# HengyiWang/MorpheuS

Hardware: AMD Instinct MI355X
Metric: rays/sec (fwd+bwd, 128 samples/ray) (higher is better)
Workload: dtype f32 (exact 3 x bf16 operand split on the bf16 MFMA pipe, fp32 accumulate)

## Files before the change

include/morpheus_hip.h:

```cpp
#ifndef MORPHEUS_HIP_H
#define MORPHEUS_HIP_H

#include <stdint.h>

#ifdef __cplusplus
extern "C" {
#endif

#define MH_OK 0
#define MH_ERR_ARG 1
#define MH_ERR_LAUNCH 2
#define MH_ERR_OVERFLOW 3

#define MH_ABI_VERSION 9
#define MH_MAX_LEVELS 32
#define MH_TILE 32

int mh_abi_version(void);
const char *mh_status_string(int status);

int mh_grid_encode_fwd(const float *x, const float *emb, const int32_t *offsets_host,
                       const int32_t *res_host, float *out, int64_t M, int32_t L, int32_t n_levels,
                       float bound, int32_t group, void *stream);
int mh_grid_encode_bwd(const float *grad, const float *x, const float *emb,
// ... 102 lines not shown
int64_t mh_field_wpack_floats(void);
int64_t mh_field_wpackT_floats(void);
int mh_field_fwd(const float *xc, const float *feat_s, const float *feat_c, const float *topo,
                 const float *wpack, const float *bias, const float *beta, int32_t n_bands, int32_t with_color,
                 float *sdf, float *sigma, float *albedo, float *acts, int64_t M, void *stream);
int64_t mh_mlp_wgrad_workspace_floats(int32_t n_layers, const int32_t *in_feats_host,
                                      const int32_t *out_feats_host, int64_t n_tiles);
int mh_mlp_wgrad(const float *acts, const float *dpre, int64_t acts_tile_floats, int64_t dpre_tile_floats,
                 int32_t n_layers, const int32_t *act_off_host, const int32_t *dpre_off_host,
                 const int32_t *in_feats_host, const int32_t *out_feats_host, const int32_t *in_live_host,
                 const int32_t *out_live_host, float *workspace, float *dw_raw, float *db_raw, int64_t n_tiles, void *stream);
int mh_mlp_wgrad_b3(const float *acts, const float *dpre, int64_t acts_tile_floats, int64_t dpre_tile_floats,
                    int32_t n_layers, const int32_t *act_off_host, const int32_t *dpre_off_host,
                    const int32_t *in_feats_host, const int32_t *out_feats_host, const int32_t *in_live_host,
                    const int32_t *out_live_host, float *workspace, float *dw_raw, float *db_raw, int64_t n_tiles, void *stream);

int mh_weight_norm_fwd(int32_t n_layers, const float *const *v_host, const float *const *g_host, float *const *w_host,
                       const int32_t *rows_host, const int32_t *cols_host, void *stream);
int mh_weight_norm_bwd(int32_t n_layers, const float *const *v_host, const float *const *g_host,
                       const float *const *dw_host, float *const *dv_host, float *const *dg_host,
                       const int32_t *rows_host, const int32_t *cols_host, void *stream);

int64_t mh_field_bwd_fused_workspace_floats(int64_t M);
int64_t mh_field_dgeo_floats(int64_t M);
int mh_field_bwd_fused(const float *xc, const float *sdf, const float *albedo, const float *g_sdf, const float *g_sigma,
                       const float *g_albedo, const float *wpackT, const float *beta, int32_t n_bands, int32_t with_color,
                       const float *acts, float *dgeo_scratch, float *workspace, float *raw, int32_t accumulate, float *g_xc,
                       float *g_feat_s, float *g_feat_c, float *g_topo, uint32_t *gmax_bits, int64_t M, void *stream);
int64_t mh_field_w3T_bytes(void);
int mh_field_bwd_fused_b3(const float *xc, const float *sdf, const float *albedo, const float *g_sdf, const float *g_sigma,
                          const float *g_albedo, const void *w3T, const float *beta, int32_t n_bands, int32_t with_color,
                          const float *acts, float *dgeo_scratch, float *workspace, float *raw, int32_t accumulate, float *g_xc,
                          float *g_feat_s, float *g_feat_c, float *g_topo, uint32_t *gmax_bits, int64_t M, void *stream);
int mh_adam_step(float *params, const float *grads, float *exp_avg, float *exp_avg_sq, int64_t n, int32_t n_segs,
                 const int64_t *seg_end_host, const float *seg_lr_host, const int64_t *seg_step_host, float beta1,
                 float beta2, float eps, void *stream);
int mh_adam_step_dev(float *params, const float *grads, float *exp_avg, float *exp_avg_sq, int64_t n, int32_t n_segs,
                     const int64_t *seg_end_host, const float *seg_lr_host, const float *seg_flag_dev, int64_t *seg_step_dev,
                     float *seg_scratch_dev, float beta1, float beta2, float eps, void *stream);

int64_t mh_masked_mean_workspace_floats(void);
int mh_masked_mean_fwd(int32_t kind, const float *a, const float *b, const float *w_row, int64_t M, int32_t C,
                       const int32_t *n_valid, float *ws, float *out, void *stream);
int mh_masked_mean_bwd(int32_t kind, const float *a, const float *b, const float *w_row, int64_t M, int32_t C,
                       const int32_t *n_valid, const float *out, const float *g, float *g_a, float *g_b, void *stream);
int mh_ortho_perturb_fwd(const float *x, const float *n, const float *phi, float scale, int64_t M, float *out, void *stream);
int mh_ortho_perturb_bwd(const float *n, const float *phi, const float *g_out, float scale, int64_t M, float *g_n, void *stream);
int mh_smooth_points_fwd(const float *depth, const float *off, const float *rays_o, const float *rays_d, int64_t N, int32_t K,
                         float *pts, float *keep, void *stream);
int mh_smooth_points_bwd(const float *g_pts, const float *depth, const float *off, const float *rays_d, int64_t N, int32_t K,
                         float *g_depth, float *g_o, float *g_d, void *stream);
int mh_bg_blend_fwd(const float *color, const float *opacity, const float *bg, int64_t N, float *image, void *stream);
int mh_bg_blend_bwd(const float *g_image, const float *opacity, const float *bg, int64_t N, float *g_opacity, float *g_bg, void *stream);

int64_t mh_pose_bwd_workspace_floats(int64_t B, int64_t n_per_row);
int mh_pose_apply_fwd(const float *rays_o, const float *rays_d, const float *pose, const int64_t *frame_of_row, int64_t B,
                      int64_t n_per_row, float *o_out, float *d_out, void *stream);
int mh_pose_apply_bwd(const float *rays_d, const float *pose, const int64_t *frame_of_row, int64_t B, int64_t n_per_row,
                      int64_t n_frames, const float *g_o, const float *g_d, float *ws, float *g_pose, void *stream);

int mh_render_loss_fwd(const float *pred_rgb, const float *pred_depth, const float *opacity, const float *image,
                       const float *depth, const float *mask, const float *bg, const float *rays_o, const float *rays_d,
                       int64_t N, float w_rgb, float w_mask, float w_depth, float *gt_rgb, float *valid, float *out, void *stream);
int mh_render_loss_bwd(const float *pred_rgb, const float *pred_depth, const float *opacity, const float *gt_rgb,
                       const float *depth, const float *mask, const float *valid, int64_t N, float w_rgb, float w_mask,
                       float w_depth, const float *g, float *g_rgb, float *g_depth, float *g_opacity, void *stream);
// ... 98 lines not shown
```

morpheus_amd/csrc/mlp.hip:

```cpp
#include "mlp_dev.h"
#include <stdlib.h>


__shared__ f32x4 lds_w[4096];

template <int N_F4>
__device__ __forceinline__ void stage_weights(const float *__restrict__ g) {
    static_assert(N_F4 % 256 == 0, "whole rounds of the 256-thread block");
    __syncthreads();
    const f32x4 *src = reinterpret_cast<const f32x4 *>(g);
    const int wave = threadIdx.x >> 6;
#pragma unroll
    for (int k = 0; k < N_F4 / 256; k++)
        __builtin_amdgcn_global_load_lds((const __attribute__((address_space(1))) void *)(src + k * 256 + threadIdx.x),
                                         (__attribute__((address_space(3))) void *)(lds_w + k * 256 + wave * 64), 16, 0, 0);
    asm volatile("s_waitcnt vmcnt(0)" ::: "memory");
    __syncthreads();
}

template <int N_F4>
__device__ __forceinline__ void stage_issue(const float *__restrict__ g) {
    static_assert(N_F4 % 256 == 0, "whole rounds of the 256-thread block");
    const f32x4 *src = reinterpret_cast<const f32x4 *>(g);
    const int wave = threadIdx.x >> 6;
#pragma unroll
    for (int k = 0; k < N_F4 / 256; k++)
        __builtin_amdgcn_global_load_lds((const __attribute__((address_space(1))) void *)(src + k * 256 + threadIdx.x),
                                         (__attribute__((address_space(3))) void *)(lds_w + k * 256 + wave * 64), 16, 0, 0);
}
__device__ __forceinline__ void stage_wait() {
    asm volatile("s_waitcnt vmcnt(0)" ::: "memory");
    __syncthreads();
}

// ... 1043 lines not shown
                wsdf[mt] += q[(7 + mt) * 64 + lane];
            }
            gb_acc += q[6 * 64 + lane];
        }
    }
    if (wave != 0) return;
#pragma unroll
    for (int o = 32; o > 0; o >>= 1) gb_acc += __shfl_xor(gb_acc, o);
    if (lane == 0) ws[part.gb + blockIdx.x] = gb_acc;
    const int64_t pchunk = blockIdx.x;
#pragma unroll
    for (int mt = 0; mt < 2; mt++) {
        dw_store<3>(ws + part.dw[0] + pchunk * 64 * 96, w0[mt], mt, 96, i, h);
        dw_store<2>(ws + part.dw[1] + pchunk * 64 * 64, w1[mt], mt, 64, i, h);
    }
    {
        f32x16 z[2];
        acc_zero<2>(z);
        if (!WITH_COLOR) dw_store<2>(ws + part.dw[2] + pchunk * 64 * 64, z, 0, 64, i, h);
        if (h == 0) {
            z[0][0] = wsdf[0];
            z[1][0] = wsdf[1];
        }
        dw_store<2>(ws + part.dw[2] + pchunk * 64 * 64, z, 1, 64, i, h);
    }
    if (h == 0) {
        if (!WITH_COLOR) ws[part.db[2] + pchunk * 64 + i] = 0.f;
        ws[part.db[2] + pchunk * 64 + 32 + i] = i == 0 ? bsdf : 0.f;
#pragma unroll
        for (int mt = 0; mt < 2; mt++) {
            ws[part.db[1] + pchunk * 64 + 32 * mt + i] = b1[mt];
            ws[part.db[0] + pchunk * 64 + 32 * mt + i] = b0[mt];
        }
    }
}

template <int IT>
struct WgFrag {
    f32x4 a[4];
    f32x4 b[IT][4];
};

__device__ __forceinline__ int wg_row(int row, int live) { return row < live ? row : live - 1; }

template <int IT>
__device__ __forceinline__ void wg_load(WgFrag<IT> &f, const float *__restrict__ acts, const float *__restrict__ dpre,
                                        int64_t t, int64_t acts_tile_floats, int64_t dpre_tile_floats, int act_off,
                                        int dpre_off, int mt, int i, int h, int in_live, int out_live) {
    const f32x4 *a = reinterpret_cast<const f32x4 *>(dpre + t * dpre_tile_floats + dpre_off + (int64_t)wg_row(32 * mt + i, out_live) * TILE + 16 * h);
#pragma unroll
    for (int j = 0; j < 4; j++) f.a[j] = a[j];
#pragma unroll
    for (int n = 0; n < IT; n++) {
        const f32x4 *b = reinterpret_cast<const f32x4 *>(acts + t * acts_tile_floats + act_off + (int64_t)wg_row(32 * n + i, in_live) * TILE + 16 * h);
#pragma unroll
        for (int j = 0; j < 4; j++) f.b[n][j] = b[j];
    }
}

template <int IT>
__device__ __forceinline__ void wg_load_async(WgFrag<IT> &f, const float *__restrict__ acts, const float *__restrict__ dpre,
                                              int64_t t, int64_t acts_tile_floats, int64_t dpre_tile_floats, int act_off,
                                              int dpre_off, int mt, int i, int h, int in_live, int out_live) {
    const float *a = dpre + t * dpre_tile_floats + dpre_off + (int64_t)wg_row(32 * mt + i, out_live) * TILE + 16 * h;
    asm volatile("global_load_dwordx4 %0, %1, off" : "=v"(f.a[0]) : "v"(a) : "memory");
    asm volatile("global_load_dwordx4 %0, %1, off offset:16" : "=v"(f.a[1]) : "v"(a) : "memory");
// ... 888 lines not shown
    const WarpWg w = warp_wg_geometry();
    WgRegenHost rg;
    for (int k = 0; k < WG_MAX_LAYERS; k++) rg.on[k] = false;
    rg.M = M;
    for (int net = 0; net < 2; net++) {
        const int k = net * 6 + 4;
        rg.on[k] = regen_dpre4 != 0;
        rg.g5[k] = net ? g_topo : g_deform;
        rg.nout[k] = net ? 2 : 3;
        rg.w3T[k] = reinterpret_cast<const f32x4 *>(net ? w3T_t : w3T_d);
        rg.mask_off[k] = WARP_HID_ROWS * TILE + (net * 5 + 4) * 64 * 2;
    }
    return wgrad_impl(acts, dpre, (int64_t)WARP_ACT_ROWS * TILE, (int64_t)WARP_DPRE_ROWS * TILE, 12, w.act_off, w.dpre_off, w.in, w.out,
                      w.in_live, w.out_live, workspace, dw_raw, db_raw, n_tiles_for(M), stream, true, regen_dpre4 ? &rg : nullptr);
}

static const int FUSED_IN[6] = {96, 64, 64, 64, 64, 64};
static const int FUSED_OUT[6] = {64, 64, 64, 64, 64, 32};

static inline int fused_blocks(int64_t n_tiles) {
    const int64_t need = (n_tiles + FUSED_THREADS / 64 - 1) / (FUSED_THREADS / 64);
    const int64_t cus = mh_cu_count();
    return (int)(need < cus ? need : cus);
}

extern "C" int64_t mh_field_bwd_fused_workspace_floats(int64_t M) {
    const int64_t chunks = (int64_t)fused_blocks(n_tiles_for(M));
    int64_t per = 0;
    for (int l = 0; l < 6; l++) per += (int64_t)FUSED_IN[l] * FUSED_OUT[l] + FUSED_OUT[l];
    return chunks * (per + 1);
}
extern "C" int64_t mh_field_dgeo_floats(int64_t M) { return n_tiles_for(M) * 64 * 16; }

static int field_bwd_fused_impl(const float *xc, const float *sdf, const float *albedo, const float *g_sdf,
                                const float *g_sigma, const float *g_albedo, const float *wpackT, const float *beta,
                                int32_t n_bands, int32_t with_color, const float *acts, float *dgeo_scratch,
                                float *workspace, float *raw, int32_t accumulate, float *g_xc, float *g_feat_s, float *g_feat_c,
                                float *g_topo, uint32_t *gmax_bits, int64_t M, void *stream, bool b3) {
    if (M == 0) return MH_OK;
    if (M < 0 || !xc || !sdf || !wpackT || !acts || !workspace || !raw || n_bands < 0 || n_bands > 6 || !beta) return MH_ERR_ARG;
    if (with_color && (!albedo || !dgeo_scratch)) return MH_ERR_ARG;
    static MhOncePerDevice opted;
    const size_t lds_c = (size_t)(FUSED_TC2(b3) + FUSED_TC1(b3) + FUSED_TC0(b3)) * 16 + (size_t)(4 * SCR_FLOATS) * sizeof(float);
    const size_t lds_s = (size_t)(FUSED_TS2(b3) + FUSED_TS1(b3) + FUSED_TS0(b3)) * 16 + (size_t)(4 * SCR_FLOATS) * sizeof(float);
    const int dev = mh_device();
    if (opted.need(dev)) {
        const int big_c = (int)((size_t)(FUSED_TC2(1) + FUSED_TC1(1) + FUSED_TC0(1)) * 16 + (size_t)(4 * SCR_FLOATS) * sizeof(float));
        const int big_s = (int)((size_t)(FUSED_TS2(1) + FUSED_TS1(1) + FUSED_TS0(1)) * 16 + (size_t)(4 * SCR_FLOATS) * sizeof(float));
        if (hipFuncSetAttribute((const void *)field_fused_color_kernel<false>, hipFuncAttributeMaxDynamicSharedMemorySize, big_c) != hipSuccess ||
            hipFuncSetAttribute((const void *)field_fused_color_kernel<true>, hipFuncAttributeMaxDynamicSharedMemorySize, big_c) != hipSuccess ||
            hipFuncSetAttribute((const void *)field_fused_sdf_kernel<true, false>, hipFuncAttributeMaxDynamicSharedMemorySize, big_s) != hipSuccess ||
            hipFuncSetAttribute((const void *)field_fused_sdf_kernel<false, false>, hipFuncAttributeMaxDynamicSharedMemorySize, big_s) != hipSuccess ||
            hipFuncSetAttribute((const void *)field_fused_sdf_kernel<true, true>, hipFuncAttributeMaxDynamicSharedMemorySize, big_s) != hipSuccess ||
            hipFuncSetAttribute((const void *)field_fused_sdf_kernel<false, true>, hipFuncAttributeMaxDynamicSharedMemorySize, big_s) != hipSuccess)
            return MH_ERR_LAUNCH;
        opted.mark(dev);
    }
    const int64_t n_tiles = n_tiles_for(M);
    const int blocks = fused_blocks(n_tiles);
    const int64_t chunks = blocks;
    int64_t dw_off[6], db_off[6], off = 0, dw_total = 0, db_total = 0;
    for (int l = 0; l < 6; l++) {
        dw_off[l] = off;
        off += chunks * FUSED_IN[l] * FUSED_OUT[l];
        dw_total += (int64_t)FUSED_IN[l] * FUSED_OUT[l];
    }
    for (int l = 0; l < 6; l++) {
        db_off[l] = off;
        off += chunks * FUSED_OUT[l];
        db_total += FUSED_OUT[l];
    }
    FusedPart pc, ps;
    for (int k = 0; k < 3; k++) {
        ps.dw[k] = dw_off[k];
        ps.db[k] = db_off[k];
        pc.dw[k] = dw_off[3 + k];
        pc.db[k] = db_off[3 + k];
    }
    ps.gb = off;
    pc.gb = off;
    ps.dw_s2 = pc.dw_s2 = dw_off[2];
    ps.db_s2 = pc.db_s2 = db_off[2];
    hipStream_t st = mh_stream(stream);
#define FUSED_LAUNCH_COLOR(B3_)                                                                                             \
    hipLaunchKernelGGL(field_fused_color_kernel<B3_>, dim3((unsigned)blocks), dim3(FUSED_THREADS), lds_c, st, albedo, g_albedo, wpackT, \
                       acts, dgeo_scratch, g_feat_c, workspace, pc, gmax_bits, M, n_tiles)
#define FUSED_LAUNCH_SDF(WC, B3_, DGEO)                                                                                      \
    hipLaunchKernelGGL((field_fused_sdf_kernel<WC, B3_>), dim3((unsigned)blocks), dim3(FUSED_THREADS), lds_s, st, xc, sdf, g_sdf, \
                       g_sigma, wpackT, beta, (int)n_bands, acts, (const float *)(DGEO), g_xc, g_feat_s, g_topo,             \
                       workspace, ps, gmax_bits, M, n_tiles)
    if (with_color) {
        if (b3) FUSED_LAUNCH_COLOR(true); else FUSED_LAUNCH_COLOR(false);
        MH_CHECK_LAUNCH();
        if (b3) FUSED_LAUNCH_SDF(true, true, dgeo_scratch); else FUSED_LAUNCH_SDF(true, false, dgeo_scratch);
    } else {
        if (b3) FUSED_LAUNCH_SDF(false, true, nullptr); else FUSED_LAUNCH_SDF(false, false, nullptr);
    }
#undef FUSED_LAUNCH_COLOR
#undef FUSED_LAUNCH_SDF
    MH_CHECK_LAUNCH();
    const int n_l = with_color ? 6 : 3;
    WgReduce rd;
    rd.n = 13;
    rd.accumulate = accumulate ? 1 : 0;
    int64_t dw_out = 0, db_out = 0;
    rd.first[0] = 0;
    for (int l = 0; l < 6; l++) {
        const int32_t ch = l < n_l ? (int32_t)chunks : 0;
        rd.chunks[l] = ch;
        rd.len[l] = FUSED_IN[l] * FUSED_OUT[l];
        rd.part_off[l] = dw_off[l];
        rd.out_off[l] = dw_out;
        rd.chunks[6 + l] = ch;
        rd.len[6 + l] = FUSED_OUT[l];
        rd.part_off[6 + l] = db_off[l];
        rd.out_off[6 + l] = dw_total + db_out;
        dw_out += (int64_t)FUSED_IN[l] * FUSED_OUT[l];
        db_out += FUSED_OUT[l];
    }
    rd.chunks[12] = (int32_t)chunks;
    rd.len[12] = 1;
    rd.part_off[12] = ps.gb;
    rd.out_off[12] = dw_total + db_total;
    for (int sgm = 0; sgm < rd.n; sgm++) rd.first[sgm + 1] = rd.first[sgm] + rd.len[sgm];
// ... 39 lines not shown
```

morpheus_amd/ops.py:

```python
from __future__ import annotations

import ctypes
import math
import os
from typing import Optional, Sequence

import numpy as np
import torch

from . import _lib
from ._lib import check, launch, ptr, require_gpu, stream
from .packing import field_joint_packer, field_packer, warp_joint_packer, warp_packer



class KernelTimer:

    def __init__(self):
        self.enabled = False
        self.records = {}
        self._pool, self._used = [], 0

    def reset(self, enabled: bool):
        self.enabled, self.records, self._used = enabled, {}, 0
# ... 847 lines not shown
    for net in range(2):
        for l in range(6):
            act_off.append(0 if l == 0 else (64 + net * 640 + (l - 1) * 128) * 32)
            dpre_off.append((net * 672 + l * 128) * 32)
            in_pad.append(64 if l == 0 else 128)
            out_pad.append(32 if l == 5 else 128)
            in_live.append(40 if l == 0 else 128)
            out_live.append((3, 2)[net] if l == 5 else 128)
    return act_off, dpre_off, in_pad, out_pad, in_live, out_live


_WARP_WG = _warp_wg_geometry()

def warp_mlp(x, slot, bias0_d, bias0_t, n_bands, opnd: MLPOperands, slots_are_identity: bool = False):
    return _WarpMLP.apply(x, slot, bias0_d, bias0_t, opnd.token, n_bands, opnd, slots_are_identity)


def _field_fwd(lib, xc, fs, fc, tp, beta_c, n_bands, with_color, opnd, need_grad):
    w, b = opnd.w[0], opnd.b[0]
    M, dev = xc.shape[0], xc.device
    acts = _scratch(lib.mh_field_acts_floats(M), dev) if need_grad else None
    sdf, sigma = torch.empty(M, device=dev), torch.empty(M, device=dev)
    albedo = torch.empty(M, 3, device=dev) if with_color else None
    if opnd.w3 is not None:
        _timed("mh_field_fwd_b3", ptr(xc), ptr(fs), ptr(fc), ptr(tp), ptr(opnd.w3[0]), ptr(b), ptr(beta_c), n_bands,
               int(bool(with_color)), ptr(sdf), ptr(sigma), ptr(albedo), ptr(acts), M, key="mh_field_fwd")
    else:
        _timed("mh_field_fwd", ptr(xc), ptr(fs), ptr(fc), ptr(tp), ptr(w), ptr(b), ptr(beta_c), n_bands, int(bool(with_color)),
               ptr(sdf), ptr(sigma), ptr(albedo), ptr(acts), M)
    return sdf, sigma, albedo, acts


FIELD_BWD = os.environ.get("MORPHEUS_FIELD_BWD", "b3")
if FIELD_BWD not in ("b3", "sdf", "f32"):
    raise ValueError(f"MORPHEUS_FIELD_BWD={FIELD_BWD!r}: expected 'b3', 'sdf' or 'f32'")


def _field_wT(opnd, with_color: bool):
    sliced = FIELD_BWD == "b3" or (FIELD_BWD == "sdf" and not with_color)
    if sliced and opnd.mode == "b3" and opnd.wT3 is not None:
        return opnd.wT3[0], True
    return opnd.wT[0], False


def _field_bwd(lib, xc, wT, beta_c, acts, sdf, albedo, g_sdf, g_sigma, g_albedo, n_bands, with_color, has_topo, has_fc,
               need_dx, jp, raw_into=None, gmax=None, b3=False):
    M, dev = xc.shape[0], xc.device
    if not with_color:
        g_albedo = None
    g_xc = torch.empty(M, 3, device=dev) if need_dx else None
    g_fs = _scratch(M * 32, dev).view(M, 32)
    g_fc = _scratch(M * 32, dev).view(M, 32) if (with_color and has_fc) else None
    g_tp = torch.empty(M, 2, device=dev) if has_topo else None
    if gmax is None:
        gmax = torch.zeros(2, dtype=torch.int32, device=dev)
    dgeo = _scratch(lib.mh_field_dgeo_floats(M), dev) if with_color else None
    ws = torch.empty(lib.mh_field_bwd_fused_workspace_floats(M), device=dev)
    raw = None
    if raw_into is None:
        raw = torch.empty(jp.raw_len + 1, device=dev) if M > 0 else torch.zeros(jp.raw_len + 1, device=dev)
    c = lambda t: None if t is None else t.contiguous()
    _timed("mh_field_bwd_fused_b3" if b3 else "mh_field_bwd_fused", ptr(xc), ptr(sdf), ptr(albedo if with_color else None), ptr(c(g_sdf)),
           ptr(c(g_sigma)), ptr(c(g_albedo)), ptr(wT), ptr(beta_c), n_bands, int(with_color), ptr(acts), ptr(dgeo), ptr(ws),
           ptr(raw) if raw_into is None else ctypes.c_void_p(raw_into), int(raw_into is not None), ptr(g_xc), ptr(g_fs), ptr(g_fc),
           ptr(g_tp), ptr(gmax), M, key="mh_field_bwd_fused")
    return g_xc, g_fs, g_fc, g_tp, raw, gmax


class _FieldMLP(torch.autograd.Function):

    @staticmethod
    def forward(ctx, xc, feat_s, feat_c, topo, beta, token, n_bands, with_color, opnd):
        ctx.set_materialize_grads(False)
        require_gpu(xc, feat_s, feat_c, topo, beta)
        lib = _lib.load()
        xc = xc.detach().contiguous().float()
        fs = feat_s.detach().contiguous()
        fc = None if feat_c is None else feat_c.detach().contiguous()
        tp = None if topo is None else topo.detach().contiguous()
        beta_c = beta.detach().reshape(1).contiguous().float()
        sdf, sigma, albedo, acts = _field_fwd(lib, xc, fs, fc, tp, beta_c, n_bands, with_color, opnd, any(ctx.needs_input_grad))
        wT_sel, ctx.bwd_b3 = _field_wT(opnd, bool(with_color))
        ctx.save_for_backward(xc, wT_sel, beta_c, acts, sdf, albedo)
        ctx.cfg = (n_bands, bool(with_color), topo is not None, feat_c is not None)
        ctx.jp = opnd.jp
        if albedo is None:
            albedo = torch.empty(0, device=xc.device)
            ctx.mark_non_differentiable(albedo)
        return sdf, sigma, albedo

    @staticmethod
    def backward(ctx, g_sdf, g_sigma, g_albedo):
        lib = _lib.load()
        xc, wT, beta_c, acts, sdf, albedo = ctx.saved_tensors
# ... 388 lines not shown
```

Baseline: 1.062 million.

## Add paired-wave 512-thread field backward kernels splitting output tiles across waves

New measurement: 1.085 million (median of 6 runs). +2.1%, better.

```diff
diff --git a/include/morpheus_hip.h b/include/morpheus_hip.h
--- a/include/morpheus_hip.h
+++ b/include/morpheus_hip.h
@@ -158,6 +158,7 @@
                           const float *g_albedo, const void *w3T, const float *beta, int32_t n_bands, int32_t with_color,
                           const float *acts, float *dgeo_scratch, float *workspace, float *raw, int32_t accumulate, float *g_xc,
                           float *g_feat_s, float *g_feat_c, float *g_topo, uint32_t *gmax_bits, int64_t M, void *stream);
+int64_t mh_field_bwd_pair_min_points(int64_t set);
 int mh_adam_step(float *params, const float *grads, float *exp_avg, float *exp_avg_sq, int64_t n, int32_t n_segs,
                  const int64_t *seg_end_host, const float *seg_lr_host, const int64_t *seg_step_host, float beta1,
                  float beta2, float eps, void *stream);
diff --git a/morpheus_amd/csrc/mlp.hip b/morpheus_amd/csrc/mlp.hip
--- a/morpheus_amd/csrc/mlp.hip
+++ b/morpheus_amd/csrc/mlp.hip
@@ -1,5 +1,6 @@
 #include "mlp_dev.h"
 #include <stdlib.h>
+#include <atomic>
 
 
 __shared__ f32x4 lds_w[4096];
@@ -1109,6 +1110,606 @@
             ws[part.db[1] + pchunk * 64 + 32 * mt + i] = b1[mt];
             ws[part.db[0] + pchunk * 64 + 32 * mt + i] = b0[mt];
         }
+    }
+}
+
+#define PAIR_THREADS 512
+#define PAIR_RED_FLOATS (6 * 1024 + 8 * 64)
+
+#define PAIR_LANE_ANEW                                            \
+    int lane_anew = threadIdx.x & 63;                             \
+    asm volatile("" : "+v"(lane_anew));                           \
+    const int lane = lane_anew, pt = lane & 31, h = lane >> 5, i = lane & 31
+
+struct PairWalk {
+    int64_t chunk, n_chunks, trips;
+};
+__device__ __forceinline__ PairWalk pair_walk(int pair, int64_t n_tiles) {
+    PairWalk w;
+    w.n_chunks = 4 * (int64_t)gridDim.x;
+    const int64_t first = 4 * (int64_t)blockIdx.x;
+    w.chunk = first + pair;
+    w.trips = first < n_tiles ? (n_tiles - first + w.n_chunks - 1) / w.n_chunks : 0;
+    return w;
+}
+
+template <int N_F4>
+__device__ __forceinline__ void stage_pair(const float *__restrict__ g) {
+    const f32x4 *src = reinterpret_cast<const f32x4 *>(g);
+    for (int i = threadIdx.x; i < N_F4; i += PAIR_THREADS) lds_fused[i] = src[i];
+}
+
+__device__ __forceinline__ void scr_put_tile(float *__restrict__ scr, const float (&v)[16], int t, int pt, int h) {
+#pragma unroll
+    for (int r = 0; r < 16; r++) scr[(32 * t + acc_row(r, h)) * SCR_STRIDE + pt] = v[r];
+}
+
+template <int KS, int MT, int NT, int S_RUN = KS / 8>
+__device__ __forceinline__ void mfma_tiles_z_b3(const f32x4 *__restrict__ w, int t0, const float (&bin)[KS], f32x16 (&acc)[NT], int lane) {
+    static_assert(KS % 8 == 0 && S_RUN >= 1 && S_RUN <= KS / 8 && NT <= MT, "k16 steps");
+    constexpr int S = KS / 8, PL = MT * S * 64;
+    const f32x16 zero = {0.f, 0.f, 0.f, 0.f, 0.f, 0.f, 0.f, 0.f, 0.f, 0.f, 0.f, 0.f, 0.f, 0.f, 0.f, 0.f};
+    w += t0 * S * 64 + lane;
+#pragma unroll
+    for (int s = 0; s < S_RUN; s++) {
+        Frag bh, bm, bl;
+#pragma unroll
+        for (int e2 = 0; e2 < 4; e2++) split2(bin[8 * s + 2 * e2], bin[8 * s + 2 * e2 + 1], bh.u[e2], bm.u[e2], bl.u[e2]);
+        Frag ah[NT], am[NT], al[NT];
+#pragma unroll
+        for (int t = 0; t < NT; t++) {
+            ah[t].f = w[0 * PL + (t * S + s) * 64];
+            am[t].f = w[1 * PL + (t * S + s) * 64];
+            al[t].f = w[2 * PL + (t * S + s) * 64];
+        }
+#pragma unroll
+        for (int t = 0; t < NT; t++) acc[t] = __builtin_amdgcn_mfma_f32_32x32x16_bf16(al[t].h, bh.h, s == 0 ? zero : acc[t], 0, 0, 0);
+#pragma unroll
+        for (int t = 0; t < NT; t++) acc[t] = __builtin_amdgcn_mfma_f32_32x32x16_bf16(am[t].h, bm.h, acc[t], 0, 0, 0);
+#pragma unroll
+        for (int t = 0; t < NT; t++) acc[t] = __builtin_amdgcn_mfma_f32_32x32x16_bf16(ah[t].h, bl.h, acc[t], 0, 0, 0);
+#pragma unroll
+        for (int t = 0; t < NT; t++) acc[t] = __builtin_amdgcn_mfma_f32_32x32x16_bf16(am[t].h, bh.h, acc[t], 0, 0, 0);
+#pragma unroll
+        for (int t = 0; t < NT; t++) acc[t] = __builtin_amdgcn_mfma_f32_32x32x16_bf16(ah[t].h, bm.h, acc[t], 0, 0, 0);
+#pragma unroll
+        for (int t = 0; t < NT; t++) acc[t] = __builtin_amdgcn_mfma_f32_32x32x16_bf16(ah[t].h, bh.h, acc[t], 0, 0, 0);
+        __builtin_amdgcn_sched_barrier(0);
+    }
+}
+
+template <int MT, int NT>
+__device__ __forceinline__ void mfma_tiles_scr_b3(const f32x4 *__restrict__ w, int t0, const float *__restrict__ scr, int pt, int h,
+                                                  f32x16 (&acc)[NT], int lane) {
+    constexpr int S = 4, PL = MT * S * 64;
+    const f32x16 zero = {0.f, 0.f, 0.f, 0.f, 0.f, 0.f, 0.f, 0.f, 0.f, 0.f, 0.f, 0.f, 0.f, 0.f, 0.f, 0.f};
+    w += t0 * S * 64 + lane;
+    scr += 4 * h * SCR_STRIDE + pt;
+#pragma unroll
+    for (int s = 0; s < S; s++) {
+        float bin[8];
+#pragma unroll
+        for (int e = 0; e < 8; e++) bin[e] = scr[(32 * (s >> 1) + acc_row(8 * (s & 1) + e, 0)) * SCR_STRIDE];
+        Frag bh, bm, bl;
+#pragma unroll
+        for (int e2 = 0; e2 < 4; e2++) split2(bin[2 * e2], bin[2 * e2 + 1], bh.u[e2], bm.u[e2], bl.u[e2]);
+        Frag ah[NT], am[NT], al[NT];
+#pragma unroll
+        for (int t = 0; t < NT; t++) {
+            ah[t].f = w[0 * PL + (t * S + s) * 64];
+            am[t].f = w[1 * PL + (t * S + s) * 64];
+            al[t].f = w[2 * PL + (t * S + s) * 64];
+        }
+#pragma unroll
+        for (int t = 0; t < NT; t++) acc[t] = __builtin_amdgcn_mfma_f32_32x32x16_bf16(al[t].h, bh.h, s == 0 ? zero : acc[t], 0, 0, 0);
+#pragma unroll
+        for (int t = 0; t < NT; t++) acc[t] = __builtin_amdgcn_mfma_f32_32x32x16_bf16(am[t].h, bm.h, acc[t], 0, 0, 0);
+#pragma unroll
+        for (int t = 0; t < NT; t++) acc[t] = __builtin_amdgcn_mfma_f32_32x32x16_bf16(ah[t].h, bl.h, acc[t], 0, 0, 0);
+#pragma unroll
+        for (int t = 0; t < NT; t++) acc[t] = __builtin_amdgcn_mfma_f32_32x32x16_bf16(am[t].h, bh.h, acc[t], 0, 0, 0);
+#pragma unroll
+        for (int t = 0; t < NT; t++) acc[t] = __builtin_amdgcn_mfma_f32_32x32x16_bf16(ah[t].h, bm.h, acc[t], 0, 0, 0);
+#pragma unroll
+        for (int t = 0; t < NT; t++) acc[t] = __builtin_amdgcn_mfma_f32_32x32x16_bf16(ah[t].h, bh.h, acc[t], 0, 0, 0);
+        __builtin_amdgcn_sched_barrier(0);
+    }
+}
+
+__device__ __forceinline__ void dw_bias(const RowFrag &a, float &bsum) {
+#pragma unroll
+    for (int j = 0; j < 4; j++) bsum += (a.v[j][0] + a.v[j][1]) + (a.v[j][2] + a.v[j][3]);
+}
+template <int NI>
+__device__ __forceinline__ void dw_mfma_b3(const RowFrag &a, const RowSl *__restrict__ b, f32x16 (&acc)[NI]) {
+    RowSl as;
+    row_slices(a, as);
+#pragma unroll
+    for (int s = 0; s < 2; s++) {
+#pragma unroll
+        for (int n = 0; n < NI; n++) acc[n] = __builtin_amdgcn_mfma_f32_32x32x16_bf16(as.l[s].h, b[n].h[s].h, acc[n], 0, 0, 0);
+#pragma unroll
+        for (int n = 0; n < NI; n++) acc[n] = __builtin_amdgcn_mfma_f32_32x32x16_bf16(as.m[s].h, b[n].m[s].h, acc[n], 0, 0, 0);
+#pragma unroll
+        for (int n = 0; n < NI; n++) acc[n] = __builtin_amdgcn_mfma_f32_32x32x16_bf16(as.h[s].h, b[n].l[s].h, acc[n], 0, 0, 0);
+#pragma unroll
+        for (int n = 0; n < NI; n++) acc[n] = __builtin_amdgcn_mfma_f32_32x32x16_bf16(as.m[s].h, b[n].h[s].h, acc[n], 0, 0, 0);
+#pragma unroll
+        for (int n = 0; n < NI; n++) acc[n] = __builtin_amdgcn_mfma_f32_32x32x16_bf16(as.h[s].h, b[n].m[s].h, acc[n], 0, 0, 0);
+#pragma unroll
+        for (int n = 0; n < NI; n++) acc[n] = __builtin_amdgcn_mfma_f32_32x32x16_bf16(as.h[s].h, b[n].h[s].h, acc[n], 0, 0, 0);
+    }
+}
+__device__ __forceinline__ void dw_mfma_b3_2(const RowFrag &a, const RowSl *__restrict__ b, f32x16 &acc0, f32x16 &acc1) {
+    RowSl as;
+    row_slices(a, as);
+#pragma unroll
+    for (int s = 0; s < 2; s++) {
+        acc0 = __builtin_amdgcn_mfma_f32_32x32x16_bf16(as.l[s].h, b[0].h[s].h, acc0, 0, 0, 0);
+        acc1 = __builtin_amdgcn_mfma_f32_32x32x16_bf16(as.l[s].h, b[1].h[s].h, acc1, 0, 0, 0);
+        acc0 = __builtin_amdgcn_mfma_f32_32x32x16_bf16(as.m[s].h, b[0].m[s].h, acc0, 0, 0, 0);
+        acc1 = __builtin_amdgcn_mfma_f32_32x32x16_bf16(as.m[s].h, b[1].m[s].h, acc1, 0, 0, 0);
+        acc0 = __builtin_amdgcn_mfma_f32_32x32x16_bf16(as.h[s].h, b[0].l[s].h, acc0, 0, 0, 0);
+        acc1 = __builtin_amdgcn_mfma_f32_32x32x16_bf16(as.h[s].h, b[1].l[s].h, acc1, 0, 0, 0);
+        acc0 = __builtin_amdgcn_mfma_f32_32x32x16_bf16(as.m[s].h, b[0].h[s].h, acc0, 0, 0, 0);
+        acc1 = __builtin_amdgcn_mfma_f32_32x32x16_bf16(as.m[s].h, b[1].h[s].h, acc1, 0, 0, 0);
+        acc0 = __builtin_amdgcn_mfma_f32_32x32x16_bf16(as.h[s].h, b[0].m[s].h, acc0, 0, 0, 0);
+        acc1 = __builtin_amdgcn_mfma_f32_32x32x16_bf16(as.h[s].h, b[1].m[s].h, acc1, 0, 0, 0);
+        acc0 = __builtin_amdgcn_mfma_f32_32x32x16_bf16(as.h[s].h, b[0].h[s].h, acc0, 0, 0, 0);
+        acc1 = __builtin_amdgcn_mfma_f32_32x32x16_bf16(as.h[s].h, b[1].h[s].h, acc1, 0, 0, 0);
+    }
+}
+template <int NI>
+__device__ __forceinline__ void dw_store_at(float *__restrict__ dw, const f32x16 (&acc)[NI], int mt, int in_pad, int n0, int i, int h) {
+#pragma unroll
+    for (int n = 0; n < NI; n++)
+#pragma unroll
+        for (int r = 0; r < 16; r++) dw[(int64_t)(32 * mt + acc_row(r, h)) * in_pad + 32 * (n0 + n) + i] = acc[n][r];
+}
+
+__global__ __launch_bounds__(PAIR_THREADS, 1) void field_pair_color_kernel(
+    const float *__restrict__ albedo, const float *__restrict__ g_albedo, const float *__restrict__ wpackT,
+    const float *__restrict__ acts, float *__restrict__ dgeo_scr, float *__restrict__ g_feat_c, float *__restrict__ ws,
+    FusedPart part, uint32_t *__restrict__ gmax, int64_t M, int64_t n_tiles) {
+    const int lane = threadIdx.x & 63, wave = __builtin_amdgcn_readfirstlane(threadIdx.x >> 6);
+    const int pair = wave & 3, k = wave >> 2;
+    const int pt = lane & 31, h = lane >> 5, i = lane & 31;
+    constexpr int W_F4 = FUSED_TC2(1) + FUSED_TC1(1) + FUSED_TC0(1);
+    stage_pair<W_F4>(wpackT);
+    float *scrX = reinterpret_cast<float *>(lds_fused + W_F4) + pair * (2 * SCR_FLOATS), *scrY = scrX + SCR_FLOATS;
+    __syncthreads();
+    f32x16 w2[1], w1[2][1], w0[2][1], wg[1];
+    acc_zero<1>(w2);
+    acc_zero<1>(wg);
+#pragma unroll
+    for (int mt = 0; mt < 2; mt++) {
+        acc_zero<1>(w1[mt]);
+        acc_zero<1>(w0[mt]);
+    }
+    float b2 = 0.f, bg = 0.f;
+    float b1 = 0.f, b0 = 0.f;
+    uint32_t max_c = 0;
+    const PairWalk walk = pair_walk(pair, n_tiles);
+    RowFrag B[1];
+    for (int64_t trip = 0; trip < walk.trips; trip++) {
+        const int64_t want = walk.chunk + trip * walk.n_chunks;
+        const bool active = want < n_tiles;
+        const int64_t tile_id = active ? want : n_tiles - 1;
+        const int64_t p = tile_id * TILE + pt;
+        const bool live = active && p < M;
+        const float *atile = acts + tile_id * (int64_t)(FIELD_ACT_ROWS * TILE);
+        const uint32_t *masks = reinterpret_cast<const uint32_t *>(atile + FIELD_HID_ROWS * TILE);
+        const f32x4 *wt = lds_fused;
+        RowFrag A;
+        RowSl Bs[1];
+        f32x16 acc[1];
+        float own[16];
+        float d2[16];
+#pragma unroll
+        for (int r = 0; r < 16; r++) d2[r] = 0.f;
+        if (g_albedo && live && h == 0) {
+#pragma unroll
+            for (int c = 0; c < 3; c++) {
+                const float a = albedo[p * 3 + c];
+                d2[c] = g_albedo[p * 3 + c] * a * (1.0f - a);
+            }
+        }
+        const uint32_t mw3 = masks[3 * 64 + lane] >> (16 * k), mw2 = masks[2 * 64 + lane] >> (16 * k);
+        row_load_async(B[0], atile, 352 + 32 * k + i, h);
+        if (k == 0) scr_put<1>(scrX, d2, pt, h);
+        mfma_tiles_z_b3<16, 2, 1, 1>(wt, k, d2, acc, lane);
+        wt += FUSED_TC2(1);
+#pragma unroll
+        for (int r = 0; r < 16; r++) own[r] = mask_bit(mw3, r, acc[0][r]);
+        __syncthreads();
+        scr_get(A, scrX, i, h);
+        fused_wait<1>(B);
+        row_slices(B[0], Bs[0]);
+        if (k == 0) dw_bias(A, b2);
+        dw_mfma_b3<1>(A, Bs, w2);
+        __builtin_amdgcn_sched_barrier(0);
+        row_load_async(B[0], atile, 288 + 32 * k + i, h);
+        scr_put_tile(scrY, own, k, pt, h);
+        __syncthreads();
+        mfma_tiles_scr_b3<2, 1>(wt, k, scrY, pt, h, acc, lane);
+        wt += FUSED_TC1(1);
+#pragma unroll
+        for (int r = 0; r < 16; r++) own[r] = mask_bit(mw2, r, acc[0][r]);
+        fused_wait<1>(B);
+        row_slices(B[0], Bs[0]);
+#pragma unroll
+        for (int mt = 0; mt < 2; mt++) {
+            scr_get(A, scrY, 32 * mt + i, h);
+            if (k == mt) dw_bias(A, b1);
+            dw_mfma_b3<1>(A, Bs, w1[mt]);
+        }
+        __builtin_amdgcn_sched_barrier(0);
+        row_load_async(B[0], atile, 224 + 32 * k + i, h);
+        scr_put_tile(scrX, own, k, pt, h);
+        __syncthreads();
+        mfma_tiles_scr_b3<2, 1>(wt, k, scrX, pt, h, acc, lane);
+        if (k == 0) {
+            if (live && g_feat_c) {
+                f32x4 *o = reinterpret_cast<f32x4 *>(g_feat_c + p * 32 + 16 * h);
+#pragma unroll
+                for (int q = 0; q < 4; q++) {
+                    f32x4 v;
+#pragma unroll
+                    for (int c = 0; c < 4; c++) v[c] = acc[0][4 * q + c];
+                    o[q] = v;
+                }
+#pragma unroll
+                for (int r = 0; r < 16; r++) max_c = max(max_c, __float_as_uint(fabsf(acc[0][r])));
+            }
+        } else if (active) {
+            f32x4 *o = reinterpret_cast<f32x4 *>(dgeo_scr + (tile_id * 64 + lane) * 16);
+#pragma unroll
+            for (int q = 0; q < 4; q++) {
+                f32x4 v;
+#pragma unroll
+                for (int c = 0; c < 4; c++) v[c] = acc[0][4 * q + c];
+                o[q] = v;
+            }
+        }
+        fused_wait<1>(B);
+        row_slices(B[0], Bs[0]);
+        RowFrag Bg[1];
+        row_load_async(Bg[0], atile, 160 + 32 * k + i, h);
+#pragma unroll
+        for (int mt = 0; mt < 2; mt++) {
+            scr_get(A, scrX, 32 * mt + i, h);
+            if (k == mt) dw_bias(A, b0);
+            dw_mfma_b3<1>(A, Bs, w0[mt]);
+        }
+        __builtin_amdgcn_sched_barrier(0);
+        if (k == 1) {
+            float dg[16];
+#pragma unroll
+            for (int r = 0; r < 16; r++) dg[r] = acc[0][r];
+            scr_put<1>(scrY, dg, pt, h);
+        }
+        __syncthreads();
+        fused_wait<1>(Bg);
+        row_slices(Bg[0], Bs[0]);
+        scr_get(A, scrY, i, h);
+        if (k == 0) dw_bias(A, bg);
+        dw_mfma_b3<1>(A, Bs, wg);
+        __builtin_amdgcn_sched_barrier(0);
+    }
+    if (gmax) {
+#pragma unroll
+        for (int o = 32; o > 0; o >>= 1) max_c = max(max_c, (uint32_t)__shfl_xor((int)max_c, o));
+        if (lane == 0 && max_c) atomicMax(gmax + 1, max_c);
+    }
+    bg += __shfl_xor(bg, 32);
+    b2 += __shfl_xor(b2, 32);
+    b1 += __shfl_xor(b1, 32);
+    b0 += __shfl_xor(b0, 32);
+    float *red = reinterpret_cast<float *>(lds_fused) + k * PAIR_RED_FLOATS;
+    for (int src = 1; src < 4; src++) {
+        __syncthreads();
+        if (pair == src) {
+            float *q = acc_to_lds<1>(w2, red, lane);
+            q = acc_to_lds<1>(w1[0], q, lane);
+            q = acc_to_lds<1>(w1[1], q, lane);
+            q = acc_to_lds<1>(w0[0], q, lane);
+            q = acc_to_lds<1>(w0[1], q, lane);
+            q = acc_to_lds<1>(wg, q, lane);
+            q[0 * 64 + lane] = b2;
+            q[1 * 64 + lane] = b1;
+            q[2 * 64 + lane] = b0;
+            q[3 * 64 + lane] = bg;
+        }
+        __syncthreads();
+        if (pair == 0) {
+            const float *q = acc_add_lds<1>(w2, red, lane);
+            q = acc_add_lds<1>(w1[0], q, lane);
+            q = acc_add_lds<1>(w1[1], q, lane);
+            q = acc_add_lds<1>(w0[0], q, lane);
+            q = acc_add_lds<1>(w0[1], q, lane);
+            q = acc_add_lds<1>(wg, q, lane);
+            b2 += q[0 * 64 + lane];
+            b1 += q[1 * 64 + lane];
+            b0 += q[2 * 64 + lane];
+            bg += q[3 * 64 + lane];
+        }
+    }
+    if (pair != 0) return;
+    const int64_t pchunk = blockIdx.x;
+    dw_store_at<1>(ws + part.dw[2] + pchunk * 32 * 64, w2, 0, 64, k, i, h);
+#pragma unroll
+    for (int mt = 0; mt < 2; mt++) {
+        dw_store_at<1>(ws + part.dw[1] + pchunk * 64 * 64, w1[mt], mt, 64, k, i, h);
+        dw_store_at<1>(ws + part.dw[0] + pchunk * 64 * 64, w0[mt], mt, 64, k, i, h);
+    }
+    dw_store_at<1>(ws + part.dw_s2 + pchunk * 64 * 64, wg, 0, 64, k, i, h);
+    if (h == 0) {
+        if (k == 0) {
+            ws[part.db[2] + pchunk * 32 + i] = b2;
+            ws[part.db_s2 + pchunk * 64 + i] = bg;
+        }
+        ws[part.db[1] + pchunk * 64 + 32 * k + i] = b1;
+        ws[part.db[0] + pchunk * 64 + 32 * k + i] = b0;
+    }
+}
+
+__global__ __launch_bounds__(PAIR_THREADS, 1) void field_pair_sdf_kernel(
+    const float *__restrict__ xc, const float *__restrict__ sdf, const float *__restrict__ g_sdf,
+    const float *__restrict__ g_sigma, const float *__restrict__ wpackT, const float *__restrict__ beta_p, int n_bands,
+    const float *__restrict__ acts, const float *__restrict__ dgeo_scr, float *__restrict__ g_xc,
+    float *__restrict__ g_feat_s, float *__restrict__ g_topo, float *__restrict__ ws,
+    FusedPart part, uint32_t *__restrict__ gmax, int64_t M, int64_t n_tiles) {
+    const int wave = __builtin_amdgcn_readfirstlane(threadIdx.x >> 6);
+    const int pair = wave & 3, k = wave >> 2;
+    constexpr int W_F4 = FUSED_TS2(1) + FUSED_TS1(1) + FUSED_TS0(1);
+    stage_pair<W_F4>(wpackT + 4 * (FUSED_TC2(1) + FUSED_TC1(1) + FUSED_TC0(1)));
+    float *scrX = reinterpret_cast<float *>(lds_fused + W_F4) + pair * (2 * SCR_FLOATS), *scrY = scrX + SCR_FLOATS;
+    __syncthreads();
+    f32x16 w1[2][1], wa[2][1], wb[2];
+    acc_zero<2>(wb);
+#pragma unroll
+    for (int mt = 0; mt < 2; mt++) {
+        acc_zero<1>(w1[mt]);
+        acc_zero<1>(wa[mt]);
+    }
+    float wsdf = 0.f;
+    float bsdf = 0.f, gb_acc = 0.f;
+    float b1 = 0.f, b0 = 0.f;
+    uint32_t max_s = 0;
+    const float beta = *beta_p;
+    const float half_ib2 = __int_as_float(__builtin_amdgcn_readfirstlane(__float_as_int(0.5f / (beta * beta))));
+    const float one_ib2 = __int_as_float(__builtin_amdgcn_readfirstlane(__float_as_int(1.0f / (beta * beta))));
+    const float one_ib = __int_as_float(__builtin_amdgcn_readfirstlane(__float_as_int(1.0f / beta)));
+    const PairWalk walk = pair_walk(pair, n_tiles);
+    RowFrag B[2];
+    for (int64_t trip = 0; trip < walk.trips; trip++) {
+        const int64_t want = walk.chunk + trip * walk.n_chunks;
+        const bool active = want < n_tiles;
+        const int64_t tile_id = active ? want : n_tiles - 1;
+        PAIR_LANE_ANEW;
+        const int64_t p = tile_id * TILE + pt;
+        const bool live = active && p < M;
+        const float *atile = acts + tile_id * (int64_t)(FIELD_ACT_ROWS * TILE);
+        const uint32_t *masks = reinterpret_cast<const uint32_t *>(atile + FIELD_HID_ROWS * TILE);
+        const f32x4 *wt = lds_fused;
+        RowFrag A;
+        f32x16 acc[1];
+        float own[16];
+        float gs = 0.f, gbeta = 0.f;
+        if (live && h == 0) {
+            const float s = sdf[p];
+            if (g_sdf) gs = g_sdf[p];
+            if (g_sigma) {
+                const float gsg = g_sigma[p];
+                const float sg = (s > 0.f) ? 1.f : ((s < 0.f) ? -1.f : 0.f);
+                const float a = fabsf(s) / beta;
+                const float ex = expf(-a);
+                gs += gsg * (-half_ib2 * sg * sg * ex);
+                gbeta = gsg * (-one_ib2 * laplace_unit(s, beta) + one_ib * (0.5f * sg * ex * (fabsf(s) / (beta * beta))));
+            }
+        }
+        gb_acc += gbeta;
+        const uint32_t mw1 = masks[1 * 64 + lane] >> (16 * k), mw0 = masks[0 * 64 + lane] >> (16 * k);
+        float d2[32];
+        {
+            const f32x4 *gsrc = reinterpret_cast<const f32x4 *>(dgeo_scr + (tile_id * 64 + lane) * 16);
+#pragma unroll
+            for (int q = 0; q < 4; q++) {
+                const f32x4 v = gsrc[q];
+#pragma unroll
+                for (int c = 0; c < 4; c++) d2[4 * q + c] = active ? v[c] : 0.f;
+            }
+        }
+#pragma unroll
+        for (int r = 0; r < 16; r++) d2[16 + r] = 0.f;
+        d2[16] = gs;
+        row_load_async(B[0], atile, 160 + 32 * k + i, h);
+        mfma_tiles_z_b3<32, 2, 1, 3>(wt, k, d2, acc, lane);
+        wt += FUSED_TS2(1);
+#pragma unroll
+        for (int r = 0; r < 16; r++) own[r] = mask_bit(mw1, r, acc[0][r]);
+        fused_wait<1>(B);
+#pragma unroll
+        for (int j = 0; j < 4; j++)
+#pragma unroll
+            for (int q = 0; q < 4; q++) {
+                const float g = __shfl(gs, 16 * h + 4 * j + q);
+                wsdf = fmaf(g, B[0].v[j][q], wsdf);
+                bsdf += g;
+            }
+        asm volatile("" : "+v"(wsdf), "+v"(bsdf));
+        __builtin_amdgcn_sched_barrier(0);
+        {
+            PAIR_LANE_ANEW;
+            RowSl Bs[1];
+            row_load_async(B[0], atile, 96 + 32 * k + i, h);
+            scr_put_tile(scrX, own, k, pt, h);
+            __syncthreads();
+            mfma_tiles_scr_b3<2, 1>(wt, k, scrX, pt, h, acc, lane);
+            wt += FUSED_TS1(1);
+#pragma unroll
+            for (int r = 0; r < 16; r++) own[r] = mask_bit(mw0, r, acc[0][r]);
+            fused_wait<1>(B);
+            row_slices(B[0], Bs[0]);
+#pragma unroll
+            for (int mt = 0; mt < 2; mt++) {
+                scr_get(A, scrX, 32 * mt + i, h);
+                if (k == mt) dw_bias(A, b1);
+                dw_mfma_b3<1>(A, Bs, w1[mt]);
+            }
+            __builtin_amdgcn_sched_barrier(0);
+        }
+        {
+            PAIR_LANE_ANEW;
+            row_load_async(B[0], atile, k == 0 ? 64 + min(i, 15) : i, h);
+            row_load_async(B[1], atile, k == 0 ? 64 + min(i, 15) : 32 + i, h);
+            scr_put_tile(scrY, own, k, pt, h);
+        }
+        __syncthreads();
+        if (k == 0) {
+            PAIR_LANE_ANEW;
+            const int64_t p = tile_id * TILE + pt;
+            const bool live = active && p < M;
+            RowSl Bs[1];
+            f32x16(&e)[2] = wb;
+            mfma_tiles_scr_b3<3, 2>(wt, 0, scrY, pt, h, e, lane);
+            float gx[3] = {0.f, 0.f, 0.f};
+            if (g_xc) {
+                float dsc[18];
+                enc_deriv_parked(atile, pt, h, dsc);
+#pragma unroll
+                for (int kk = 0; kk < 18; kk++) {
+                    const float de = kk < 16 ? e[0][kk] : e[1][kk - 16];
+                    gx[kk % 3] += de * dsc[kk];
+                }
+                if (h == 0) {
+                    gx[0] += e[1][2];
+                    gx[2] += e[1][3];
+                } else {
+                    gx[1] += e[1][2];
+                }
+#pragma unroll
+                for (int d = 0; d < 3; d++) gx[d] += __shfl_xor(gx[d], 32);
+            }
+            if (live) {
+                if (g_xc && h == 0) {
+                    g_xc[p * 3 + 0] = gx[0];
+                    g_xc[p * 3 + 1] = gx[1];
+                    g_xc[p * 3 + 2] = gx[2];
+                }
+                if (g_topo) g_topo[p * 2 + h] = e[1][4];
+            }
+            __builtin_amdgcn_sched_barrier(0);
+            fused_wait<2>(B);
+            row_slices(B[0], Bs[0]);
+#pragma unroll
+            for (int mt = 0; mt < 2; mt++) {
+                scr_get(A, scrY, 32 * mt + i, h);
+                if (mt == 0) dw_bias(A, b0);
+                dw_mfma_b3<1>(A, Bs, wa[mt]);
+                __builtin_amdgcn_sched_barrier(0);
+            }
+            __builtin_amdgcn_sched_barrier(0);
+        } else {
+            PAIR_LANE_ANEW;
+            const int64_t p = tile_id * TILE + pt;
+            const bool live = active && p < M;
+            RowSl Bs[2];
+            f32x16 e[1];
+            mfma_tiles_scr_b3<3, 1>(wt, 2, scrY, pt, h, e, lane);
+            if (live && g_feat_s) {
+                f32x4 *o = reinterpret_cast<f32x4 *>(g_feat_s + p * 32 + 16 * h);
+#pragma unroll
+                for (int q = 0; q < 4; q++) {
+                    f32x4 v;
+#pragma unroll
+                    for (int c = 0; c < 4; c++) v[c] = e[0][4 * q + c];
+                    o[q] = v;
+                }
+#pragma unroll
+                for (int r = 0; r < 16; r++) max_s = max(max_s, __float_as_uint(fabsf(e[0][r])));
+            }
+            __builtin_amdgcn_sched_barrier(0);
+            fused_wait<2>(B);
+            row_slices(B[0], Bs[0]);
+            row_slices(B[1], Bs[1]);
+#pragma unroll
+            for (int mt = 0; mt < 2; mt++) {
+                scr_get(A, scrY, 32 * mt + i, h);
+                if (mt == 1) dw_bias(A, b0);
+                dw_mfma_b3_2(A, Bs, wa[mt][0], wb[mt]);
+                __builtin_amdgcn_sched_barrier(0);
+            }
+            __builtin_amdgcn_sched_barrier(0);
+        }
+    }
+    const int lane = __lane_id(), h = lane >> 5, i = lane & 31;
+    if (gmax) {
+#pragma unroll
+        for (int o = 32; o > 0; o >>= 1) max_s = max(max_s, (uint32_t)__shfl_xor((int)max_s, o));
+        if (lane == 0 && max_s) atomicMax(gmax + 0, max_s);
+    }
+    wsdf += __shfl_xor(wsdf, 32);
+    bsdf += __shfl_xor(bsdf, 32);
+    b1 += __shfl_xor(b1, 32);
+    b0 += __shfl_xor(b0, 32);
+    float *red = reinterpret_cast<float *>(lds_fused) + k * PAIR_RED_FLOATS;
+    for (int src = 1; src < 4; src++) {
+        __syncthreads();
+        if (pair == src) {
+            float *q = acc_to_lds<1>(w1[0], red, lane);
+            q = acc_to_lds<1>(w1[1], q, lane);
+            q = acc_to_lds<1>(wa[0], q, lane);
+            q = acc_to_lds<1>(wa[1], q, lane);
+            if (k == 1) acc_to_lds<2>(wb, q, lane);
+            q += 2 * 1024;
+            q[0 * 64 + lane] = bsdf;
+            q[1 * 64 + lane] = b1;
+            q[2 * 64 + lane] = b0;
+            q[3 * 64 + lane] = wsdf;
+            q[4 * 64 + lane] = gb_acc;
+        }
+        __syncthreads();
+        if (pair == 0) {
+            const float *q = acc_add_lds<1>(w1[0], red, lane);
+            q = acc_add_lds<1>(w1[1], q, lane);
+            q = acc_add_lds<1>(wa[0], q, lane);
+            q = acc_add_lds<1>(wa[1], q, lane);
+            if (k == 1) acc_add_lds<2>(wb, q, lane);
+            q += 2 * 1024;
+            bsdf += q[0 * 64 + lane];
+            b1 += q[1 * 64 + lane];
+            b0 += q[2 * 64 + lane];
+            wsdf += q[3 * 64 + lane];
+            gb_acc += q[4 * 64 + lane];
+        }
+    }
+    if (pair != 0) return;
+    const int64_t pchunk = blockIdx.x;
+    if (k == 0) {
+#pragma unroll
+        for (int o = 32; o > 0; o >>= 1) gb_acc += __shfl_xor(gb_acc, o);
+        if (lane == 0) ws[part.gb + blockIdx.x] = gb_acc;
+    }
+#pragma unroll
+    for (int mt = 0; mt < 2; mt++) {
+        dw_store_at<1>(ws + part.dw[1] + pchunk * 64 * 64, w1[mt], mt, 64, k, i, h);
+        dw_store_at<1>(ws + part.dw[0] + pchunk * 64 * 96, wa[mt], mt, 96, k == 0 ? 2 : 0, i, h);
+        if (k == 1) {
+            const f32x16(&w)[1] = reinterpret_cast<const f32x16(&)[1]>(wb[mt]);
+            dw_store_at<1>(ws + part.dw[0] + pchunk * 64 * 96, w, mt, 96, 1, i, h);
+        }
+    }
+    {
+        f32x16 z[1];
+        acc_zero<1>(z);
+        if (h == 0) z[0][0] = wsdf;
+        dw_store_at<1>(ws + part.dw[2] + pchunk * 64 * 64, z, 1, 64, k, i, h);
+    }
+    if (h == 0) {
+        if (k == 0) ws[part.db[2] + pchunk * 64 + 32 + i] = i == 0 ? bsdf : 0.f;
+        ws[part.db[1] + pchunk * 64 + 32 * k + i] = b1;
+        ws[part.db[0] + pchunk * 64 + 32 * k + i] = b0;
     }
 }
 
@@ -2063,6 +2664,12 @@
 }
 extern "C" int64_t mh_field_dgeo_floats(int64_t M) { return n_tiles_for(M) * 64 * 16; }
 
+static std::atomic<int64_t> g_pair_min_points{0};
+extern "C" int64_t mh_field_bwd_pair_min_points(int64_t set) {
+    if (set >= 0) g_pair_min_points.store(set, std::memory_order_relaxed);
+    return g_pair_min_points.load(std::memory_order_relaxed);
+}
+
 static int field_bwd_fused_impl(const float *xc, const float *sdf, const float *albedo, const float *g_sdf,
                                 const float *g_sigma, const float *g_albedo, const float *wpackT, const float *beta,
                                 int32_t n_bands, int32_t with_color, const float *acts, float *dgeo_scratch,
@@ -2074,6 +2681,10 @@
     static MhOncePerDevice opted;
     const size_t lds_c = (size_t)(FUSED_TC2(b3) + FUSED_TC1(b3) + FUSED_TC0(b3)) * 16 + (size_t)(4 * SCR_FLOATS) * sizeof(float);
     const size_t lds_s = (size_t)(FUSED_TS2(b3) + FUSED_TS1(b3) + FUSED_TS0(b3)) * 16 + (size_t)(4 * SCR_FLOATS) * sizeof(float);
+    const size_t pair_lds_c = (size_t)(FUSED_TC2(1) + FUSED_TC1(1) + FUSED_TC0(1)) * 16 + (size_t)(8 * SCR_FLOATS) * sizeof(float);
+    const size_t pair_lds_s = (size_t)(FUSED_TS2(1) + FUSED_TS1(1) + FUSED_TS0(1)) * 16 + (size_t)(8 * SCR_FLOATS) * sizeof(float);
+    static_assert((FUSED_TS2(1) + FUSED_TS1(1) + FUSED_TS0(1)) * 16 + 8 * SCR_FLOATS * 4 <= 160 * 1024, "pair form: LDS of one CU");
+    const bool pair = b3 && with_color && M >= g_pair_min_points.load(std::memory_order_relaxed);
     const int dev = mh_device();
     if (opted.need(dev)) {
         const int big_c = (int)((size_t)(FUSED_TC2(1) + FUSED_TC1(1) + FUSED_TC0(1)) * 16 + (size_t)(4 * SCR_FLOATS) * sizeof(float));
@@ -2083,7 +2694,9 @@
             hipFuncSetAttribute((const void *)field_fused_sdf_kernel<true, false>, hipFuncAttributeMaxDynamicSharedMemorySize, big_s) != hipSuccess ||
             hipFuncSetAttribute((const void *)field_fused_sdf_kernel<false, false>, hipFuncAttributeMaxDynamicSharedMemorySize, big_s) != hipSuccess ||
             hipFuncSetAttribute((const void *)field_fused_sdf_kernel<true, true>, hipFuncAttributeMaxDynamicSharedMemorySize, big_s) != hipSuccess ||
-            hipFuncSetAttribute((const void *)field_fused_sdf_kernel<false, true>, hipFuncAttributeMaxDynamicSharedMemorySize, big_s) != hipSuccess)
+            hipFuncSetAttribute((const void *)field_fused_sdf_kernel<false, true>, hipFuncAttributeMaxDynamicSharedMemorySize, big_s) != hipSuccess ||
+            hipFuncSetAttribute((const void *)field_pair_color_kernel, hipFuncAttributeMaxDynamicSharedMemorySize, (int)pair_lds_c) != hipSuccess ||
+            hipFuncSetAttribute((const void *)field_pair_sdf_kernel, hipFuncAttributeMaxDynamicSharedMemorySize, (int)pair_lds_s) != hipSuccess)
             return MH_ERR_LAUNCH;
         opted.mark(dev);
     }
@@ -2120,7 +2733,14 @@
     hipLaunchKernelGGL((field_fused_sdf_kernel<WC, B3_>), dim3((unsigned)blocks), dim3(FUSED_THREADS), lds_s, st, xc, sdf, g_sdf, \
                        g_sigma, wpackT, beta, (int)n_bands, acts, (const float *)(DGEO), g_xc, g_feat_s, g_topo,             \
                        workspace, ps, gmax_bits, M, n_tiles)
-    if (with_color) {
+    if (pair) {
+        hipLaunchKernelGGL(field_pair_color_kernel, dim3((unsigned)blocks), dim3(PAIR_THREADS), pair_lds_c, st, albedo, g_albedo, wpackT,
+                           acts, dgeo_scratch, g_feat_c, workspace, pc, gmax_bits, M, n_tiles);
+        MH_CHECK_LAUNCH();
+        hipLaunchKernelGGL(field_pair_sdf_kernel, dim3((unsigned)blocks), dim3(PAIR_THREADS), pair_lds_s, st, xc, sdf, g_sdf, g_sigma,
+                           wpackT, beta, (int)n_bands, acts, (const float *)dgeo_scratch, g_xc, g_feat_s, g_topo, workspace, ps,
+                           gmax_bits, M, n_tiles);
+    } else if (with_color) {
         if (b3) FUSED_LAUNCH_COLOR(true); else FUSED_LAUNCH_COLOR(false);
         MH_CHECK_LAUNCH();
         if (b3) FUSED_LAUNCH_SDF(true, true, dgeo_scratch); else FUSED_LAUNCH_SDF(true, false, dgeo_scratch);
diff --git a/morpheus_amd/ops.py b/morpheus_amd/ops.py
--- a/morpheus_amd/ops.py
+++ b/morpheus_amd/ops.py
@@ -903,12 +903,14 @@
 
 
 FIELD_BWD = os.environ.get("MORPHEUS_FIELD_BWD", "b3")
-if FIELD_BWD not in ("b3", "sdf", "f32"):
-    raise ValueError(f"MORPHEUS_FIELD_BWD={FIELD_BWD!r}: expected 'b3', 'sdf' or 'f32'")
+if FIELD_BWD not in ("b3", "b3w1", "sdf", "f32"):
+    raise ValueError(f"MORPHEUS_FIELD_BWD={FIELD_BWD!r}: expected 'b3', 'b3w1', 'sdf' or 'f32'")
+_PAIR_NEVER = 1 << 62
+_pair_min_default = None
 
 
 def _field_wT(opnd, with_color: bool):
-    sliced = FIELD_BWD == "b3" or (FIELD_BWD == "sdf" and not with_color)
+    sliced = FIELD_BWD in ("b3", "b3w1") or (FIELD_BWD == "sdf" and not with_color)
     if sliced and opnd.mode == "b3" and opnd.wT3 is not None:
         return opnd.wT3[0], True
     return opnd.wT[0], False
@@ -931,6 +933,13 @@
     if raw_into is None:
         raw = torch.empty(jp.raw_len + 1, device=dev) if M > 0 else torch.zeros(jp.raw_len + 1, device=dev)
     c = lambda t: None if t is None else t.contiguous()
+    if b3 and with_color:
+        global _pair_min_default
+        if _pair_min_default is None:
+            _pair_min_default = lib.mh_field_bwd_pair_min_points(-1)
+        want = _PAIR_NEVER if FIELD_BWD == "b3w1" else _pair_min_default
+        if lib.mh_field_bwd_pair_min_points(-1) != want:
+            lib.mh_field_bwd_pair_min_points(want)
     _timed("mh_field_bwd_fused_b3" if b3 else "mh_field_bwd_fused", ptr(xc), ptr(sdf), ptr(albedo if with_color else None), ptr(c(g_sdf)),
            ptr(c(g_sigma)), ptr(c(g_albedo)), ptr(wT), ptr(beta_c), n_bands, int(with_color), ptr(acts), ptr(dgeo), ptr(ws),
            ptr(raw) if raw_into is None else ctypes.c_void_p(raw_into), int(raw_into is not None), ptr(g_xc), ptr(g_fs), ptr(g_fc),
```
